# nikkolasg/playsnark

Hardware: AMD Instinct MI355X
Metric: G1 scalar-muls/s (Pippenger MSM, 2^20 pts per GPU) (higher is better)
Workload: dtype i32x14 (381-bit Fp, 28-bit unsaturated limbs, Montgomery); 1 GPU; BLS12-381 G1 MSM, 2^20 points per GPU, uniform 255-bit scalars; points_per_gpu=1048576, window_bits=20, windows=13, window_table=True, window_table_bytes=1744830464, slice=32, in_flight=4

## Files before the change

### include/playsnark_hip.h

```cpp
#ifndef PLAYSNARK_HIP_H
#define PLAYSNARK_HIP_H
#include <stddef.h>
#include <stdint.h>

#ifdef __cplusplus
extern "C" {
#endif

#define PS_OK 0
#define PS_ERR_LENGTH (-1)
#define PS_ERR_NOT_DIVISIBLE (-2)
#define PS_ERR_ENCODING (-3)
#define PS_ERR_HIP (-4)
#define PS_ERR_ARG (-5)
#define PS_ERR_NO_DEVICE (-6)

#define PS_FMT_AFFINE 0
#define PS_FMT_COMPRESSED 1

#define PS_G1 1
#define PS_G2 2

typedef struct ps_ctx ps_ctx;
typedef struct ps_points ps_points;
// ... 50 lines not shown
int ps_points_sum(int group, const uint8_t* pts, size_t k, uint8_t* out);
int ps_points_lincomb(int group, const uint8_t* pts, const uint8_t* scalars_be32, size_t k, uint8_t* out);
int ps_msm_multi_device(ps_ctx* const* ctxs, const ps_points* const* pts, const ps_scalars* const* scalars, size_t ndev, uint8_t* out);
typedef struct {
    int window_bits;
    int windows;
    uint64_t entries;
    uint64_t buckets;
    int slice;
    int window_table;
} ps_msm_info;
int ps_msm_last_info(ps_ctx* ctx, ps_msm_info* out);
int ps_msm_set_window(ps_ctx* ctx, int window_bits );
int ps_msm_set_slice(ps_ctx* ctx, int entries );
int ps_msm_set_tail(ps_ctx* ctx, int mode);
int ps_microbench_mad(ps_ctx* ctx, double* lane_mads_per_s);
#define PS_MSM_STAGES 7
int ps_ctx_set_timing(ps_ctx* ctx, int enable);
int ps_msm_last_stage_ms(ps_ctx* ctx, float ms[PS_MSM_STAGES]);

typedef struct {
    const uint32_t* row_ptr;
    const uint32_t* col;
    const int64_t* val;
} ps_csr;
int ps_qap_create(ps_ctx* ctx, size_t n_gates, size_t n_vars, size_t n_io, const ps_csr* L, const ps_csr* R,
                  const ps_csr* O, ps_qap** out);
void ps_qap_free(ps_qap* q);
typedef struct {
    const uint32_t* row_ptr;
// ... 159 lines not shown
```

### playsnark_amd/_lib.py

```python
from __future__ import annotations

import ctypes as C
import os

from .build import library_path

PS_OK = 0
PS_ERR_LENGTH = -1
PS_ERR_NOT_DIVISIBLE = -2
PS_ERR_ENCODING = -3
PS_ERR_HIP = -4
PS_ERR_ARG = -5
PS_ERR_NO_DEVICE = -6
PS_FMT_AFFINE, PS_FMT_COMPRESSED = 0, 1
PS_G1, PS_G2 = 1, 2

SYMBOLS = [
    "ps_abi_version", "ps_last_error", "ps_version", "ps_device_count",
    "ps_ctx_create", "ps_ctx_destroy", "ps_ctx_sync", "ps_ctx_stream", "ps_ctx_set_tables", "ps_ctx_set_table_budget",
    "ps_points_upload", "ps_points_from_scalars", "ps_points_download", "ps_points_download_fmt", "ps_points_len", "ps_points_group",
    "ps_points_slice", "ps_points_free", "ps_points_check_subgroup", "ps_points_precompute", "ps_points_table_window",
    "ps_scalars_upload", "ps_scalars_upload_i64", "ps_scalars_from_device_be32", "ps_scalars_download",
    "ps_scalars_len", "ps_scalars_slice", "ps_scalars_free",
    "ps_msm", "ps_msm_be32", "ps_msm_i64", "ps_msm_launch", "ps_msm_finish", "ps_msm_multi", "ps_points_sum", "ps_point_convert",
    "ps_msm_last_info", "ps_msm_set_window", "ps_msm_set_slice", "ps_msm_set_tail", "ps_microbench_mad", "ps_ctx_set_timing", "ps_msm_last_stage_ms",
    "ps_qap_create", "ps_qap_free", "ps_qap_quotient", "ps_qap_is_valid", "ps_qap_interpolate", "ps_poly_mul",
    "ps_points_lincomb", "ps_msm_multi_device", "ps_groth16_prove_multi", "ps_points_monomial_to_lagrange",
    "ps_groth16_setup", "ps_phgr13_setup", "ps_phgr13_crs_free", "ps_groth16_prove", "ps_groth16_prove_shard", "ps_groth16_prove_local", "ps_phgr13_prove", "ps_phgr13_prove_shard", "ps_phgr13_prove_multi", "ps_groth16_verify", "ps_phgr13_verify", "ps_pairing_equal", "ps_prove_last_phase_ms",
    "ps_pairing_product_is_one", "ps_groth16_verify_batch", "ps_groth16_verify_batch_locate", "ps_groth16_verify_batch_locate_info",
    "ps_qap_column_sums", "ps_groth16_setup_from_srs", "ps_groth16_crs_contribute", "ps_groth16_crs_check_update",
    "ps_scalars_powers", "ps_groth16_srs_contribute", "ps_groth16_srs_check", "ps_groth16_srs_check_update",
    "ps_points_lagrange_check", "ps_groth16_crs_check_from_srs",
    "ps_qap_create_fr", "ps_qap_wide_entries",
    "ps_msm_batch", "ps_msm_batch_set_chunk", "ps_groth16_prove_batch",
]


PS_MSM_QUEUE = 4


class MsmInfo(C.Structure):
    _fields_ = [("window_bits", C.c_int), ("windows", C.c_int), ("entries", C.c_uint64),
                ("buckets", C.c_uint64), ("slice", C.c_int), ("window_table", C.c_int)]


class VerifyLocateInfo(C.Structure):
    _fields_ = [("checks", C.c_uint32), ("levels", C.c_uint32), ("invalid", C.c_uint32), ("reserved", C.c_uint32)]


# ... 116 lines not shown
    lib.ps_msm.argtypes = [vp, vp, vp, C.c_char_p]
    lib.ps_msm_be32.argtypes = [vp, vp, C.c_char_p, sz, C.c_char_p]
    lib.ps_msm_i64.argtypes = [vp, vp, vp, sz, C.c_char_p]
    lib.ps_msm_launch.argtypes = [vp, vp, vp]
    lib.ps_msm_finish.argtypes = [vp, C.c_char_p]
    lib.ps_msm_multi.argtypes = [vp, C.POINTER(vp), C.c_size_t, vp, C.POINTER(vp)]
    lib.ps_msm_batch.argtypes = [vp, vp, vp, sz, C.c_char_p]
    lib.ps_msm_batch_set_chunk.argtypes = [vp, i]
    lib.ps_points_sum.argtypes = [i, C.c_char_p, sz, C.c_char_p]
    lib.ps_point_convert.argtypes = [i, i, i, C.c_char_p, C.c_char_p]
    lib.ps_msm_last_info.argtypes = [vp, C.POINTER(MsmInfo)]
    lib.ps_msm_set_window.argtypes = [vp, i]
    lib.ps_ctx_set_timing.argtypes = [vp, i]
    lib.ps_msm_set_slice.argtypes = [vp, i]
    lib.ps_msm_set_tail.argtypes = [vp, i]
    lib.ps_microbench_mad.argtypes = [vp, C.POINTER(C.c_double)]
    lib.ps_ctx_set_table_budget.argtypes = [vp, C.c_longlong]
    lib.ps_qap_is_valid.argtypes = [vp, vp, vp, C.POINTER(C.c_int)]
    lib.ps_msm_last_stage_ms.argtypes = [vp, C.POINTER(C.c_float)]
    lib.ps_qap_create.argtypes = [vp, sz, sz, sz, C.POINTER(Csr), C.POINTER(Csr), C.POINTER(Csr), pp]
    lib.ps_qap_create_fr.argtypes = [vp, sz, sz, sz, C.POINTER(CsrFr), C.POINTER(CsrFr), C.POINTER(CsrFr), pp]
    lib.ps_qap_wide_entries.argtypes = [vp, C.POINTER(sz)]
    lib.ps_qap_free.argtypes = [vp]
    lib.ps_qap_free.restype = None
    lib.ps_qap_quotient.argtypes = [vp, vp, vp, pp, pp, pp, pp]
    lib.ps_poly_mul.argtypes = [vp, vp, vp, pp]
    lib.ps_qap_interpolate.argtypes = [vp, vp, vp, i, pp]
    lib.ps_points_lincomb.argtypes = [i, C.c_char_p, C.c_char_p, sz, C.c_char_p]
    lib.ps_points_monomial_to_lagrange.argtypes = [vp, vp, vp, i, C.POINTER(vp)]
    lib.ps_msm_multi_device.argtypes = [C.POINTER(vp), C.POINTER(vp), C.POINTER(vp), sz, C.c_char_p]
# ... 45 lines not shown
```

### playsnark_amd/api.py

```python
from __future__ import annotations

import ctypes as C
import operator
from typing import Iterable, Optional, Sequence

from . import _lib
from ._lib import PS_G1, PS_G2, lib

G1, G2 = PS_G1, PS_G2
R_ORDER = 0x73EDA753299D7D483339D80809A1D80553BDA402FFFE5BFEFFFFFFFF00000001
FMT_AFFINE, FMT_COMPRESSED = _lib.PS_FMT_AFFINE, _lib.PS_FMT_COMPRESSED
_WIRE = {PS_G1: 96, PS_G2: 192}


class PlaysnarkError(RuntimeError):
    def __init__(self, code, msg):
        super().__init__(f"playsnark_hip error {code}: {msg}")
        self.code = code


class LengthMismatch(ValueError):
    """panic(fmt.Sprintf("mismatch of length between poly %d and blinded eval points %d")) algebra.go:351"""


# ... 41 lines not shown
        v = C.c_double(0.0)
        _check(lib.ps_microbench_mad(self._h, C.byref(v)))
        return v.value

    def set_table_budget(self, nbytes: int):
        _check(lib.ps_ctx_set_table_budget(self._h, nbytes))

    def set_slice(self, entries: int):
        _check(lib.ps_msm_set_slice(self._h, entries))

    def set_batch_chunk(self, members: int):
        _check(lib.ps_msm_batch_set_chunk(self._h, members))

    def set_tail(self, mode: int):
        _check(lib.ps_msm_set_tail(self._h, mode))

    STAGES = ("digits", "scan", "scatter", "queue", "accumulate", "fixup", "reduce")

    def set_timing(self, enable: bool):
        _check(lib.ps_ctx_set_timing(self._h, int(enable)))

    def last_stage_ms(self) -> dict:
        ms = (C.c_float * len(self.STAGES))()
        _check(lib.ps_msm_last_stage_ms(self._h, ms))
        return dict(zip(self.STAGES, list(ms)))

    def last_prove_phase_ms(self) -> dict:
        ms = (C.c_float * 4)()
        _check(lib.ps_prove_last_phase_ms(self._h, ms))
        return dict(zip(("quotient", "prep_or_h_sum", "sums", "total"), list(ms)))
# ... 799 lines not shown
```

### playsnark_amd/csrc/capi.hip

```cpp
#include "../../include/playsnark_hip.h"

#include <hip/hip_runtime.h>

#include <algorithm>
#include <atomic>
#include <chrono>
#include <condition_variable>
#include <functional>
#include <mutex>
#include <cstdio>
#include <cstring>
#include <future>
#include <string>
#include <thread>
#include <vector>

#include "msm.hpp"
#include "msm_batch.hpp"
#include "msm_batch_plan.hpp"
#include "quotient.hpp"
#include "lagrange.hpp"
#include "ec_spmv.hpp"
#include "prove_batch.hpp"
#include "share_ranges.hpp"
// ... 44 lines not shown
        if (p) (void)hipFree(p);
        p = nullptr;
        cap = 0;
    }
};

constexpr size_t PS_PINNED_SLOT = 64 * sizeof(Xyzz<Fp2>) + 16;

struct ps_ctx {
    int device = 0;
    hipStream_t stream = nullptr;
    hipStream_t tail = nullptr;
    hipEvent_t ev_acc_local = nullptr, ev_tail_done = nullptr, ev_sort_local = nullptr;
    bool tail_used = false;
    DevBuf counts, offs, bsum, keys, ranks, vals, sorted, buckets, parts, segs, wins, heavy, hparts, coarse;
    DevBuf mb_fold, mb_out;
    int batch_chunk = 0;
    hipEvent_t mb_ev[2] = {nullptr, nullptr};
    DevBuf pb_x, pb_y, pb_small;
    hipEvent_t pb_ev[6] = {nullptr, nullptr, nullptr, nullptr, nullptr, nullptr};
    bool pb_timed = false;
    DevBuf affine_tmp;
    DevBuf staging;
    DevBuf vb_f12, vb_xyzz, vb_rho, vb_cols;
    float vb_ms[6] = {0, 0, 0, 0, 0, 0};
    DevBuf lc_f12, lc_pts, lc_rows, lc_iolp, lc_work;
    ps_verify_locate_info lc_info{0, 0, 0, 0};
    float lc_ms[3] = {0, 0, 0};
    u32 simds = 0;
    struct ps_scalars* up_scalars = nullptr;
// ... 10 lines not shown
    int q_head = 0, q_len = 0;
    bool pending = false;
    ps_ctx *pipe = nullptr, *pipe2 = nullptr, *pipe3 = nullptr, *pipe4 = nullptr, *pipe5 = nullptr;
    hipEvent_t ev_fork = nullptr;
    ps_ctx* last_chain = nullptr;
    ps_ctx* last_timed = nullptr;
    float phase_ms[PS_PROVE_PHASES] = {0, 0, 0, 0};
    bool use_tables = true;
    long long table_budget = -1;
    void* d_small = nullptr;
    hipEvent_t ev_q = nullptr;
    ps_msm_info last_info{};
    int forced_c = 0;
    int forced_slice = 0;
    int forced_tail = 0;
    QuotientCache* qcache = nullptr;
    ps_ctx* aux = nullptr;
    unsigned long long g16_key[4] = {0, 0, 0, 0};
    uint8_t g16_fixed[96 * 3 + 192 * 2] = {0};
    ps_points *g16_pa = nullptr, *g16_pb = nullptr, *g16_pc = nullptr;
    bool g16_tabs = false;
    bool g16_split = false;
    size_t g16_b1_min_n = (size_t)1 << 19;
    bool g16_multi_hsplit = true;
    hipEvent_t g16_ready = nullptr;
    unsigned long long phgr_key[3] = {0, 0, 0};
    ps_points* phgr_bsum = nullptr;
    bool timing = false;
    hipEvent_t ev[PS_MSM_STAGES + 1] = {};
    bool ev_valid = false;
// ... 105 lines not shown
    }
    HIP_TRY(hipMalloc((void**)&c->d_flag, 64));
    c->h_pinned_cap = PS_MSM_MULTI_MAX * PS_PINNED_SLOT + 64;
    HIP_TRY(hipHostMalloc(&c->h_pinned, c->h_pinned_cap));
    for (auto& e : c->ev) HIP_TRY(hipEventCreate(&e));
    *out = c;
    return PS_OK;
}

extern "C" void ps_ctx_destroy(ps_ctx* c) {
    if (!c) return;
    (void)hipSetDevice(c->device);
    (void)hipStreamSynchronize(c->stream);
    if (c->tail) (void)hipStreamSynchronize(c->tail);
    for (DevBuf* b : {&c->counts, &c->offs, &c->bsum, &c->keys, &c->ranks, &c->sorted, &c->buckets, &c->parts,
                      &c->segs, &c->wins, &c->heavy, &c->hparts, &c->vals, &c->coarse, &c->staging, &c->affine_tmp, &c->mb_fold, &c->mb_out, &c->pb_x, &c->pb_y, &c->pb_small, &c->fb_table[0], &c->fb_table[1],
                      &c->vb_f12, &c->vb_xyzz, &c->vb_rho, &c->vb_cols,
                      &c->lc_f12, &c->lc_pts, &c->lc_rows, &c->lc_iolp, &c->lc_work})
        b->release();
    quotient_cache_free(c->qcache);
    if (c->up_scalars) ps_scalars_free(c->up_scalars);
    for (ps_scalars* v : c->pv_scalars)
        if (v) ps_scalars_free(v);
    if (c->g16_pa) ps_points_free(c->g16_pa);
    if (c->g16_pb) ps_points_free(c->g16_pb);
    if (c->g16_pc) ps_points_free(c->g16_pc);
    if (c->g16_ready) (void)hipEventDestroy(c->g16_ready);
    if (c->phgr_bsum) ps_points_free(c->phgr_bsum);
    if (c->aux) ps_ctx_destroy(c->aux);
    if (c->pipe) ps_ctx_destroy(c->pipe);
    if (c->pipe2) ps_ctx_destroy(c->pipe2);
// ... 737 lines not shown
            int bin_shift = 4;
            while ((pl.NB >> bin_shift) > (u32)DIGITS_BINS) bin_shift++;
            hipLaunchKernelGGL(k_digits_grouped, dgrid, dim3(DIGITS_THREADS), 2 * DIGITS_CHUNK * sizeof(u32), st, scalars_ptr(sc),
                               (u32)n, pl.c, pl.W, pl.NB, cadd, bin_shift, fold_neg, single, (u32*)c->counts.p, (u32*)c->keys.p,
                               (u32*)c->vals.p, (u32*)c->ranks.p);
        }
        PS_STAGE_MARK();
        hipLaunchKernelGGL(k_scan_blocks, dim3(scan_tiles), dim3(SCAN_BLOCK), 0, st, (const u32*)c->counts.p, (u32*)c->offs.p,
                           (u32*)c->bsum.p, (u64)G);
        hipLaunchKernelGGL(k_scan_top, dim3(1), dim3(1024), 0, st, (u32*)c->bsum.p, scan_tiles, (u32*)c->offs.p + G);
        hipLaunchKernelGGL(k_scan_add, dim3(scan_tiles), dim3(SCAN_BLOCK), 0, st, (u32*)c->offs.p, (const u32*)c->bsum.p, (u64)G);
        PS_STAGE_MARK();
        hipLaunchKernelGGL(k_scatter, dim3(nblocks(total)), dim3(256), 0, st, (const u32*)c->keys.p, (const u32*)c->vals.p,
                           (const u32*)c->ranks.p, (const u32*)c->offs.p, total, (u32*)c->sorted.p);
    }
    PS_STAGE_MARK();
    HIP_TRY(hipGetLastError());
    if (!pl.qtail) HIP_TRY(hipMemcpyAsync((char*)c->h_pinned + c->h_pinned_cap - 8, (u32*)c->offs.p + G, 4, hipMemcpyDeviceToHost, st));
    return PS_OK;
}

struct TableRef { const char* base; u64 stride; };
static bool table_ref(const ps_points* pts, size_t n, int wbits, int W, TableRef* out) {
    const Storage* st = pts->st;
    const size_t rb = table_row_bytes(pts->group);
    if (const void* t = st->table.load(std::memory_order_acquire)) {
        if (st->table_c == wbits && W <= st->table_W) {
            *out = TableRef{(const char*)t + pts->first * rb, (u64)st->table_stride};
            return true;
        }
// ... 48 lines not shown
    const bool split_fixup = !pl.shortsum;
#endif
    const size_t max_chain = split_fixup ? (size_t)nthreads_acc / 2 + 2 : 0;
    if ((rc = wc->heavy.ensure(4 * (2 * max_heavy + 3 + max_chain)))) return rc;
    const u32 heavy_npb = 256 / QTraits<KF>::GL;
    const size_t max_jobs = (size_t)nthreads_acc / heavy_npb + max_heavy + 1;
    if ((rc = wc->hparts.ensure(sizeof(Xyzz<F>) * max_jobs))) return rc;
    if (!dev_sets && sizeof(Xyzz<F>) * (pl.sets > 1 ? (size_t)pl.sets : (size_t)nres) + 16 > PS_PINNED_SLOT) return fail(PS_ERR_ARG, "too many windows");
    hipStream_t st = wc->stream;
    int evi = 4;
    if (wc->tail_used) HIP_TRY(hipStreamWaitEvent(st, wc->ev_tail_done, 0));
    if (storage_wait_ready(pts->st, st)) return fail(PS_ERR_HIP, "msm: event wait failed");
    if (wait_acc) HIP_TRY(hipStreamWaitEvent(st, wait_acc, 0));
    PS_STAGE_MARK();
    constexpr bool PF = LN == 1 || PS_G2_ACC_WAVES == 1;
    hipLaunchKernelGGL((k_accumulate<KF, PF>), dim3(nblocks((size_t)nthreads_acc * LN)), dim3(256), 0, st, src,
                       (const u32*)c->sorted.p, (const u32*)c->offs.p, (u32)G, pl.M, nthreads_acc, idx_mask, w_stride, pstride,
                       (Xyzz<F>*)wc->buckets.p, (Xyzz<F>*)wc->parts.p, (u32*)wc->heavy.p);
    if (acc_done) HIP_TRY(hipEventRecord(acc_done, st));
    PS_STAGE_MARK();
    HIP_TRY(hipEventRecord(wc->ev_acc_local, st));
    if (!inline_tail) {
        st = wc->tail;
        HIP_TRY(hipStreamWaitEvent(st, wc->ev_acc_local, 0));
    }
    if (pl.shortsum && pl.lpb >= 1) {
        const u32 lpb = qlpb;
        hipLaunchKernelGGL(k_qfixup<KF>, dim3(nblocks(G * (u64)lpb * QTraits<KF>::GL)), dim3(256), 0, st, (const u32*)c->offs.p, (u32)G, pl.M,
                           nthreads_acc, lpb, (const Xyzz<F>*)wc->parts.p, (Xyzz<F>*)wc->buckets.p, (u32*)wc->heavy.p, (u32*)wc->heavy.p + 2);
    } else if (split_fixup) {
        u32* ccount = (u32*)wc->heavy.p + 1;
        u32* clist = (u32*)wc->heavy.p + 2 + 2 * max_heavy + 1;
        hipLaunchKernelGGL(k_fixup_classify<KF>, dim3(nblocks(G * LN)), dim3(256), 0, st, (const u32*)c->offs.p, (u32)G, pl.M, nthreads_acc,
                           (Xyzz<F>*)wc->buckets.p, (u32*)wc->heavy.p, (u32*)wc->heavy.p + 2, ccount, clist);
        if (nthreads_acc > 1)
            hipLaunchKernelGGL(k_fixup_pair<KF>, dim3(nblocks((size_t)(nthreads_acc - 1) * LN)), dim3(256), 0, st, (const u32*)c->offs.p, (u32)G,
                               pl.M, nthreads_acc, (const Xyzz<F>*)wc->parts.p, (Xyzz<F>*)wc->buckets.p);
        constexpr u32 chain_npb = 256 / QTraits<KF>::GL;
        hipLaunchKernelGGL(k_qfixup_chain<KF>, dim3((unsigned)std::min<size_t>((max_chain + chain_npb - 1) / chain_npb, 512)), dim3(256), 0, st,
                           (const u32*)c->offs.p, (u32)G, pl.M, nthreads_acc, (const Xyzz<F>*)wc->parts.p, (Xyzz<F>*)wc->buckets.p,
                           (const u32*)ccount, (const u32*)clist);
    } else
    hipLaunchKernelGGL(k_fixup<KF>, dim3(nblocks(G * LN)), dim3(256), 0, st, (const u32*)c->offs.p, (u32)G, pl.M, nthreads_acc,
                       (const Xyzz<F>*)wc->parts.p, (Xyzz<F>*)wc->buckets.p, (u32*)wc->heavy.p, (u32*)wc->heavy.p + 2);
    {
        const u32* hcount = (const u32*)wc->heavy.p;
        const u32* hlist = hcount + 2;
        u32* job_base = (u32*)wc->heavy.p + 2 + max_heavy;
        hipLaunchKernelGGL(k_heavy_jobs, dim3(1), dim3(256), 0, st, (const u32*)c->offs.p, (u32)G, pl.M, nthreads_acc, hcount, hlist, job_base, heavy_npb);
        hipLaunchKernelGGL(k_qfixup_heavy_part<KF>, dim3(1024), dim3(256), 0, st, (const u32*)c->offs.p, (u32)G, pl.M, nthreads_acc,
                           (const Xyzz<F>*)wc->parts.p,
                           hcount, hlist, (const u32*)job_base, (Xyzz<F>*)wc->hparts.p);
        hipLaunchKernelGGL(k_qfixup_heavy<KF>, dim3(256), dim3(256), 0, st, (const Xyzz<F>*)wc->hparts.p, (Xyzz<F>*)wc->buckets.p, hcount,
                           hlist, (const u32*)job_base);
    }
    PS_STAGE_MARK();
    {
        Xyzz<F>* accs = (Xyzz<F>*)wc->segs.p;
        Xyzz<F>* runs = accs + nseg_total;
        Xyzz<F>* lvl = runs + nseg_total;
// ... 142 lines not shown
        }
    }
    MsmPlan pl = tab ? msm_plan_table(n, max_bits, tab_c) : msm_plan(n, max_bits, c->forced_c);
    if (tab && k == 1) {
        const MsmPlan plain = msm_plan(n, max_bits, 0);
        const double cost_tab = (double)n * pl.W * 10.0 + (double)pl.G * 42.0;
        const double cost_plain = (double)n * plain.W * 10.0 + (double)plain.G * 42.0;
        if (cost_plain < PS_TABLE_COST_MARGIN * cost_tab) pl = plain;
    }
    int plan_group = PS_G1;
    for (size_t i = 0; i < k; i++)
        if (pts[i]->group == PS_G2) plan_group = PS_G2;
    msm_plan_tail(pl, n, plan_group, c->forced_tail, c->q_len > 0);
    if (c->forced_slice) pl.M = c->forced_slice;
    if (pl.shortsum) msm_plan_lpb(pl, n, plan_group);
    if ((u64)pl.W * (u64)n >= (1ull << 32))
        return fail(PS_ERR_ARG, "MSM too long: windows x length = " + std::to_string((u64)pl.W * (u64)n) +
                                    " digits do not fit the 32-bit sort offsets (split the sum, e.g. ps_points_slice)");
    *out = pl;
    return PS_OK;
}

#ifndef PS_MULTI_CHAIN_MIN_ENTRIES
#define PS_MULTI_CHAIN_MIN_ENTRIES (1ull << 40)
#endif
#ifndef PS_CHAIN_MIN_ENTRIES
#define PS_CHAIN_MIN_ENTRIES (1ull << 21)
#endif
static int msm_launch_any(ps_ctx* wc, const ps_points* pts, const ps_scalars* sc, const MsmPlan& pl, hipEvent_t wait_acc,
                          hipEvent_t acc_done, bool inline_tail) {
// ... 39 lines not shown
    } else {
        for (int w = pl.sets - 1; w >= 0; w--) {
            for (int i = 0; i < pl.c; i++) acc = xyzz_dbl<H>(acc);
            xyzz_add<H>(acc, xyzz_to_host<F>(res[w]));
        }
    }
    write_affine(out, acc);
}

static u32 msm_entries(const ps_ctx* c, const MsmPlan& pl, int group) {
    if (!pl.qtail) return *(const u32*)((const char*)c->h_pinned + c->h_pinned_cap - 8);
    const size_t pt = group == PS_G1 ? sizeof(Xyzz<Fp>) : sizeof(Xyzz<Fp2>);
    return *(const u32*)((const char*)c->h_pinned + pt * (pl.sets > 1 ? (size_t)pl.sets : (size_t)pl.c));
}

static void write_identity(int group, uint8_t* out) {
    memset(out, 0, wire_bytes(group));
    out[0] = 0x40;
}

constexpr int PS_MULTI_RING = 4;
static int msm_multi_sort(ps_ctx* c, ps_ctx* const* ring, const ps_scalars* sc, const MsmPlan& pl, bool fork) {
    int rc;
    ps_ctx* w0 = ring[0];
    if (fork) {
        if (!c->ev_fork) HIP_TRY(hipEventCreateWithFlags(&c->ev_fork, hipEventDisableTiming));
        HIP_TRY(hipEventRecord(c->ev_fork, c->stream));
        HIP_TRY(hipStreamWaitEvent(w0->tail, c->ev_fork, 0));
    }
    if ((rc = msm_sort(w0, sc, pl, false, w0->tail))) return rc;
// ... 37 lines not shown
        }
        ring[have++] = *slots[j];
    }
    for (int j = have; j < PS_MULTI_RING; j++) ring[j] = ring[j % have];
    return PS_OK;
}

static int msm_multi_finish(ps_ctx* c, ps_ctx* w0, const ps_points* const* pts, size_t k, const MsmPlan& pl, uint8_t* const* out) {
    for (size_t i = 0; i < k; i++) {
        HIP_TRY(hipEventSynchronize(c->ev_multi[i]));
        if (!out) continue;
        if (pts[i]->group == PS_G1) msm_fold_host<Fp>(w0, pl, (int)i, out[i]);
        else msm_fold_host<Fp2>(w0, pl, (int)i, out[i]);
    }
    c->last_info = ps_msm_info{pl.c, pl.W, msm_entries(w0, pl, pts[0]->group), pl.G, pl.M, pl.table ? 1 : 0};
    return PS_OK;
}

static int msm_multi_check(const char* who, const ps_points* const* pts, size_t k, const ps_scalars* sc) {
    if (k > PS_MSM_MULTI_MAX) return fail(PS_ERR_ARG, std::string(who) + ": more than PS_MSM_MULTI_MAX point arrays");
    for (size_t i = 0; i < k; i++) {
        if (!pts[i]) return fail(PS_ERR_ARG, std::string(who) + ": NULL argument");
        if (pts[i]->n != sc->n)
            return fail(PS_ERR_LENGTH, "mismatch of length between poly " + std::to_string(sc->n) + " and blinded eval points " +
                                           std::to_string(pts[i]->n));
    }
    return PS_OK;
}

extern "C" int ps_msm_multi(ps_ctx* c, const ps_points* const* pts, size_t k, const ps_scalars* sc, uint8_t* const* out) {
// ... 35 lines not shown
        for (int j = 0; j < c->q_len; j++) busy = busy || (cand && c->q[(c->q_head + j) % PS_MSM_QUEUE].wc == cand);
        if (busy) continue;
        if (!cand) {
            int rc = ps_ctx_create(c->device, slots[w]);
            if (rc) return rc;
            cand = *slots[w];
        }
        wc = cand;
    }
    if (!wc) return fail(PS_ERR_ARG, "ps_msm_launch: no free workspace");
    if (wc != c) {
        wc->timing = c->timing;
        wc->forced_c = c->forced_c;
        wc->forced_slice = c->forced_slice;
        wc->forced_tail = c->forced_tail;
    }
    if (!c->ev_fork) HIP_TRY(hipEventCreateWithFlags(&c->ev_fork, hipEventDisableTiming));
    if (c->q_len == 0) HIP_TRY(hipEventRecord(c->ev_fork, c->stream));
    ps_ctx::PendingMsm& e = c->q[(c->q_head + c->q_len) % PS_MSM_QUEUE];
    if (sc->n == 0) {
        e = {pts->group, MsmPlan{}, wc};
    } else {
        MsmPlan pl;
        int rc0 = msm_plan_checked(c, &pts, 1, sc->n, sc->max_bits, &pl);
        if (rc0) return rc0;
        if (wc != c) HIP_TRY(hipStreamWaitEvent(wc->stream, c->ev_fork, 0));
        const bool lone = pl.shortsum && c->q_len == 0;
        if (!lone) HIP_TRY(hipStreamWaitEvent(wc->tail, c->ev_fork, 0));
        const bool chained = (u64)pl.W * sc->n >= PS_CHAIN_MIN_ENTRIES;
        hipEvent_t wait = (chained && c->last_chain && c->last_chain != wc) ? c->last_chain->ev_acc_local : nullptr;
// ... 13 lines not shown
    if (c->q_len == 0) return fail(PS_ERR_ARG, "ps_msm_finish: nothing pending");
    const ps_ctx::PendingMsm e = c->q[c->q_head];
    c->q_head = (c->q_head + 1) % PS_MSM_QUEUE;
    c->q_len--;
    c->pending = c->q_len > 0;
    const MsmPlan& pl = e.plan;
    if (pl.W == 0) {
        write_identity(e.group, out);
        return PS_OK;
    }
    HIP_TRY(hipSetDevice(c->device));
    HIP_TRY(hipEventSynchronize(e.wc->ev_tail_done));
    if (e.group == PS_G1) msm_fold_host<Fp>(e.wc, pl, 0, out);
    else msm_fold_host<Fp2>(e.wc, pl, 0, out);
    c->last_info = ps_msm_info{pl.c, pl.W, msm_entries(e.wc, pl, e.group), pl.G, pl.M, pl.table ? 1 : 0};
    c->last_timed = e.wc;
    return PS_OK;
}

extern "C" int ps_msm(ps_ctx* c, const ps_points* pts, const ps_scalars* sc, uint8_t* out) {
    if (c && c->q_len) return fail(PS_ERR_ARG, "ps_msm: sums are pending on this context (ps_msm_finish them first)");
    int rc = ps_msm_launch(c, pts, sc);
    if (rc) return rc;
    return ps_msm_finish(c, out);
}
extern "C" int ps_msm_be32(ps_ctx* c, const ps_points* pts, const uint8_t* be32, size_t n, uint8_t* out) {
    if (!c || !pts || !out || (n && !be32)) return fail(PS_ERR_ARG, "ps_msm_be32: NULL argument");
    if (c->q_len) return fail(PS_ERR_ARG, "ps_msm: sums are pending on this context (ps_msm_finish them first)");
    if (n >= (1ull << 31)) return fail(PS_ERR_ARG, "vector too long");
    HIP_TRY(hipSetDevice(c->device));
// ... 35 lines not shown
    return scope.finish(ps_msm(c, pts, s, out));
}
extern "C" int ps_msm_last_info(ps_ctx* c, ps_msm_info* out) {
    if (!c || !out) return fail(PS_ERR_ARG, "NULL argument");
    *out = c->last_info;
    return PS_OK;
}
extern "C" int ps_msm_set_slice(ps_ctx* c, int entries) {
    if (!c || entries < 0 || entries > 4096) return fail(PS_ERR_ARG, "slice must be 0 (automatic) or 1..4096");
    c->forced_slice = entries;
    return PS_OK;
}
extern "C" int ps_msm_set_tail(ps_ctx* c, int mode) {
    if (!c || mode < 0 || mode > 2) return fail(PS_ERR_ARG, "tail mode must be 0 (automatic), 1 (chains) or 2 (trees)");
    c->forced_tail = mode;
    return PS_OK;
}
extern "C" int ps_ctx_set_timing(ps_ctx* c, int enable) {
    if (!c) return fail(PS_ERR_ARG, "ctx is NULL");
    c->timing = enable != 0;
    c->ev_valid = false;
    for (ps_ctx* w : {c->pipe, c->pipe2, c->aux, c->pipe3, c->pipe4, c->pipe5})
        if (w) { w->timing = c->timing; w->ev_valid = false; }
    return PS_OK;
}
extern "C" int ps_msm_last_stage_ms(ps_ctx* c, float* ms) {
    if (!c || !ms) return fail(PS_ERR_ARG, "NULL argument");
    const ps_ctx* t = c->last_timed ? c->last_timed : c;
    if (!t->ev_valid) return fail(PS_ERR_ARG, "no timed MSM on this context (ps_ctx_set_timing)");
    HIP_TRY(hipSetDevice(c->device));
// ... 172 lines not shown
```

### playsnark_amd/csrc/msm.hpp

```cpp
#pragma once
#include "curve.hpp"
#include "fixup_class.hpp"

namespace ps {

#ifndef PS_TAIL_PRIO
#define PS_TAIL_PRIO 0
#endif
#if PS_TAIL_PRIO > 0
#define PS_TAIL_PRIO_HERE __builtin_amdgcn_s_setprio(PS_TAIL_PRIO)
#else
#define PS_TAIL_PRIO_HERE do { } while (0)
#endif

struct MsmPlan {
    int c;
    int W;
    u32 NB;
    u64 G;
    int M;
    int SEG;
    int sets;
    bool table;
    bool qtail;
    bool hybrid;
    bool shortsum;
    int lpb;
    int rc_s;
    bool busy;
};
constexpr int ENTRY_W_SHIFT = 26;

static inline MsmPlan msm_plan(size_t n, int max_bits, int forced_c) {
    MsmPlan best{};
    double best_cost = 1e300;
    for (int c = 4; c <= 20; c++) {
        if (forced_c ? c != forced_c : c > 16) continue;
        int W = max_bits / c + 1;
        double nb = (double)(1u << (c - 1));
        double cost = (double)n * W * 10.0 + W * nb * 42.0;
        if (cost < best_cost) {
            best_cost = cost;
            best.c = c;
            best.W = W;
        }
    }
    best.NB = 1u << (best.c - 1);
    best.sets = best.W;
    best.G = (u64)best.W * best.NB;
    best.M = 32;
    const u64 total = (u64)n * best.W;
    while (best.M < 1024 && total / (2 * (u64)best.M) >= (1u << 19)) best.M *= 2;
    while (best.M < 1024 && (u64)best.M * 5 * best.G < total) best.M *= 2;
    while (best.M > 8 && total / (u64)best.M < (1u << 17) && (u64)(best.M / 2) * 5 * best.G >= total) best.M /= 2;
    best.SEG = 8;
    return best;
}
static inline MsmPlan msm_plan_table(size_t n, int max_bits, int c) {
    MsmPlan pl{};
    pl.c = c;
    pl.W = max_bits / c + 1;
    pl.NB = 1u << (c - 1);
    pl.sets = 1;
    pl.table = true;
    pl.G = pl.NB;
    pl.M = 32;
    const u64 total = (u64)n * pl.W;
    while (pl.M < 1024 && total / (2 * (u64)pl.M) >= (1u << 19)) pl.M *= 2;
    while (pl.M < 1024 && (u64)pl.M * 5 * pl.G < total) pl.M *= 2;
    while (pl.M > 8 && total / (u64)pl.M < (1u << 17) && (u64)(pl.M / 2) * 5 * pl.G >= total) pl.M /= 2;
    pl.SEG = 8;
    return pl;
}

PS_INL u32 limb_sel8(const u32* k, int i) {
    u32 v = 0;
#pragma unroll
    for (int j = 0; j < 8; j++) v = (i == j) ? k[j] : v;
    return v;
}
constexpr int DIGITS_THREADS = 1024;
#ifndef PS_DIGITS_PER_THREAD
#define PS_DIGITS_PER_THREAD 8
#endif
constexpr int DIGITS_PER_THREAD = PS_DIGITS_PER_THREAD;
constexpr int DIGITS_CHUNK = DIGITS_THREADS * DIGITS_PER_THREAD;
// ... 632 lines not shown
    }
    g = lo;
    bend = offs[g + 1];
}

#ifndef PS_G2_ACC_WAVES
#define PS_G2_ACC_WAVES 2
#endif
#define PS_ACC_WAVES(KF) (FieldTraits<KF>::LANES == 2 ? PS_G2_ACC_WAVES : 2)
template <class KF, bool PREFETCH>
__global__ void __launch_bounds__(256, PS_ACC_WAVES(KF)) k_accumulate(const char* __restrict__ points,
                                                       const u32* __restrict__ sorted, const u32* __restrict__ offs,
                                                       u32 G, int Mplan, u32 T, u32 idx_mask, u64 w_stride, u32 pstride,
                                                       Xyzz<typename FieldTraits<KF>::Store>* __restrict__ buckets,
                                                       Xyzz<typename FieldTraits<KF>::Store>* __restrict__ parts,
                                                       u32* __restrict__ heavy_count) {
    const u32 E = offs[G];
    const int M = eff_slice(E, T, Mplan);
    const u32 t = logical_tid<KF>();
    if (blockIdx.x == 0 && threadIdx.x == 0) heavy_count[0] = heavy_count[1] = 0;
    const u64 start64 = (u64)t * (u64)M;
    if (start64 >= E) return;
    const u32 start = (u32)start64;
    const u32 end = (E - start < (u32)M) ? E : start + (u32)M;
    u32 lo = 0, hi = G;
    while (hi - lo > 1) {
        u32 mid = (lo + hi) >> 1;
        if (offs[mid] <= start) lo = mid; else hi = mid;
    }
    u32 g = lo;
    u32 bend = offs[g + 1];
// ... 27 lines not shown
                acc = xyzz_identity<KF>();
                run_start = p;
                next_bucket(offs, G, p, g, bend);
            }
            const u32 e = sorted[p];
            Affine<KF> pt = ld_entry_point<KF>(points, e, idx_mask, w_stride, pstride);
            if (!affine_is_identity<KF>(pt)) {
                if (e >> 31) pt.y = f_neg(pt.y);
                xyzz_madd_inl<KF>(acc, pt.x, pt.y);
            }
        }
    }
    flush_run<KF>(acc, g, run_start, end, start, t, offs, buckets, parts);
}


#ifndef PS_TAIL_WAVES
#define PS_TAIL_WAVES 2
#endif

template <class KF>
__global__ void __launch_bounds__(256, PS_TAIL_WAVES) k_fixup(const u32* __restrict__ offs, u32 G, int Mplan, u32 T,
                                                  const Xyzz<typename FieldTraits<KF>::Store>* __restrict__ parts,
                                                  Xyzz<typename FieldTraits<KF>::Store>* __restrict__ buckets,
                                                  u32* __restrict__ heavy_count, u32* __restrict__ heavy_list) {
    PS_TAIL_PRIO_HERE;
    u32 g = logical_tid<KF>();
    if (g >= G) return;
    const int M = eff_slice(offs[G], T, Mplan);
    u32 lo = offs[g], hi = offs[g + 1];
// ... 9 lines not shown
    }
    Xyzz<KF> acc = xyzz_identity<KF>();
    for (u32 t = t0; t <= t1; t++) {
        u32 slice_start = t * (u32)M;
        u32 rs = lo > slice_start ? lo : slice_start;
        Xyzz<KF> part = ld_xyzz<KF>(&parts[2 * (size_t)t + (rs == slice_start ? 0 : 1)]);
        xyzz_add_inl<KF>(acc, part);
    }
    st_xyzz<KF>(&buckets[g], acc);
}

template <class KF>
__global__ void __launch_bounds__(256) k_fixup_classify(const u32* __restrict__ offs, u32 G, int Mplan, u32 T,
                                                        Xyzz<typename FieldTraits<KF>::Store>* __restrict__ buckets,
                                                        u32* __restrict__ heavy_count, u32* __restrict__ heavy_list,
                                                        u32* __restrict__ chain_count, u32* __restrict__ chain_list) {
    PS_TAIL_PRIO_HERE;
    const u32 g = logical_tid<KF>();
    if (g >= G) return;
    const int M = eff_slice(offs[G], T, Mplan);
    const int cls = bucket_class(offs[g], offs[g + 1], (u32)M, HEAVY_SPAN);
    if (cls == BUCKET_EMPTY) {
        st_xyzz<KF>(&buckets[g], xyzz_identity<KF>());
    } else if (cls == BUCKET_CHAIN) {
        if (pair_leader<KF>()) chain_list[atomicAdd(chain_count, 1u)] = g;
    } else if (cls == BUCKET_HEAVY) {
        if (pair_leader<KF>()) heavy_list[atomicAdd(heavy_count, 1u)] = g;
    }
}

template <class KF>
__global__ void __launch_bounds__(256, PS_TAIL_WAVES) k_fixup_pair(const u32* __restrict__ offs, u32 G, int Mplan, u32 T,
                                                       const Xyzz<typename FieldTraits<KF>::Store>* __restrict__ parts,
                                                       Xyzz<typename FieldTraits<KF>::Store>* __restrict__ buckets) {
    PS_TAIL_PRIO_HERE;
    const u32 t = logical_tid<KF>() + 1;
    if (t >= T) return;
    const u32 E = offs[G];
    const int M = eff_slice(E, T, Mplan);
    u32 g;
    if (!pair_boundary_bucket(offs, G, E, t, (u32)M, HEAVY_SPAN, g)) return;
    Xyzz<KF> acc = ld_xyzz<KF>(&parts[part_slot(offs[g], t - 1, (u32)M)]);
    const Xyzz<KF> right = ld_xyzz<KF>(&parts[2 * (size_t)t]);
    xyzz_add_inl<KF>(acc, right);
    st_xyzz<KF>(&buckets[g], acc);
}

constexpr u32 HEAVY_CHUNK = 1024;
__host__ __device__ inline u32 heavy_chunk_of(u32 span, u32 npb) {
    u32 s = 1;
// ... 546 lines not shown
```

Baseline: 433.3 million G1 scalar-muls/s.

## Add whole-bucket accumulation path with size-sorted bucket ordering

```diff
diff --git a/include/playsnark_hip.h b/include/playsnark_hip.h
--- a/include/playsnark_hip.h
+++ b/include/playsnark_hip.h
@@ -88,6 +88,8 @@
 int ps_msm_set_window(ps_ctx* ctx, int window_bits );
 int ps_msm_set_slice(ps_ctx* ctx, int entries );
 int ps_msm_set_tail(ps_ctx* ctx, int mode);
+int ps_msm_set_accumulate(ps_ctx* ctx, int mode);
+int ps_msm_last_accumulate(ps_ctx* ctx, int* path);
 int ps_microbench_mad(ps_ctx* ctx, double* lane_mads_per_s);
 #define PS_MSM_STAGES 7
 int ps_ctx_set_timing(ps_ctx* ctx, int enable);
diff --git a/playsnark_amd/_lib.py b/playsnark_amd/_lib.py
--- a/playsnark_amd/_lib.py
+++ b/playsnark_amd/_lib.py
@@ -33,6 +33,7 @@
     "ps_points_lagrange_check", "ps_groth16_crs_check_from_srs",
     "ps_qap_create_fr", "ps_qap_wide_entries",
     "ps_msm_batch", "ps_msm_batch_set_chunk", "ps_groth16_prove_batch",
+    "ps_msm_set_accumulate", "ps_msm_last_accumulate",
 ]
 
 
@@ -179,6 +180,9 @@
     lib.ps_ctx_set_timing.argtypes = [vp, i]
     lib.ps_msm_set_slice.argtypes = [vp, i]
     lib.ps_msm_set_tail.argtypes = [vp, i]
+    if hasattr(lib, "ps_msm_set_accumulate"):
+        lib.ps_msm_set_accumulate.argtypes = [vp, i]
+        lib.ps_msm_last_accumulate.argtypes = [vp, C.POINTER(C.c_int)]
     lib.ps_microbench_mad.argtypes = [vp, C.POINTER(C.c_double)]
     lib.ps_ctx_set_table_budget.argtypes = [vp, C.c_longlong]
     lib.ps_qap_is_valid.argtypes = [vp, vp, vp, C.POINTER(C.c_int)]
diff --git a/playsnark_amd/api.py b/playsnark_amd/api.py
--- a/playsnark_amd/api.py
+++ b/playsnark_amd/api.py
@@ -79,6 +79,14 @@
 
     def set_tail(self, mode: int):
         _check(lib.ps_msm_set_tail(self._h, mode))
+
+    def set_accumulate(self, mode: int):
+        _check(lib.ps_msm_set_accumulate(self._h, mode))
+
+    def last_accumulate_path(self) -> int:
+        path = C.c_int(0)
+        _check(lib.ps_msm_last_accumulate(self._h, C.byref(path)))
+        return path.value
 
     STAGES = ("digits", "scan", "scatter", "queue", "accumulate", "fixup", "reduce")
 
diff --git a/playsnark_amd/csrc/bucket_order.hpp b/playsnark_amd/csrc/bucket_order.hpp
--- /dev/null
+++ b/playsnark_amd/csrc/bucket_order.hpp
@@ -0,0 +1,41 @@
+#pragma once
+#include "field.hpp"
+
+namespace ps {
+
+constexpr u32 BO_CLASSES = 256;
+constexpr u32 BO_PLACE_ITEMS = 4;
+constexpr u32 BO_PLACE_TILE = 256 * BO_PLACE_ITEMS;
+
+enum AccumulatePath : u32 { ACC_AUTO = 0, ACC_SLICES = 1, ACC_BUCKETS = 2 };
+
+constexpr u64 BO_MIN_BUCKETS = 1ull << 18;
+constexpr u64 BO_MAX_MEAN = 64;
+constexpr int BO_SHORT_BITS = 64;
+inline bool bo_host_admits(bool shortsum, u64 G, u64 digits, int max_bits) {
+    return !shortsum && max_bits > BO_SHORT_BITS && G >= BO_MIN_BUCKETS && digits <= BO_MAX_MEAN * G;
+}
+constexpr u32 BO_EVEN_MULT = 4;
+constexpr u32 BO_EVEN_ADD = 32;
+
+PS_HD inline u32 bo_class(u32 lo, u32 hi) {
+    const u32 s = hi - lo;
+    return s < BO_CLASSES - 1 ? s : BO_CLASSES - 1;
+}
+
+PS_HD inline u32 bo_scan_desc(const u32* hist, u32* start) {
+    u32 run = 0, maxc = 0;
+    for (u32 k = BO_CLASSES; k-- > 0;) {
+        start[k] = run;
+        run += hist[k];
+        if (hist[k] && k > maxc) maxc = k;
+    }
+    return maxc;
+}
+
+PS_HD inline u32 bo_verdict(u32 maxc, u32 nonempty, u32 E) {
+    if (nonempty == 0 || maxc >= BO_CLASSES - 1) return ACC_SLICES;
+    return (u64)maxc * nonempty <= (u64)BO_EVEN_MULT * E + (u64)BO_EVEN_ADD * nonempty ? ACC_BUCKETS : ACC_SLICES;
+}
+
+}
diff --git a/playsnark_amd/csrc/capi.hip b/playsnark_amd/csrc/capi.hip
--- a/playsnark_amd/csrc/capi.hip
+++ b/playsnark_amd/csrc/capi.hip
@@ -82,6 +82,7 @@
     hipEvent_t ev_acc_local = nullptr, ev_tail_done = nullptr, ev_sort_local = nullptr;
     bool tail_used = false;
     DevBuf counts, offs, bsum, keys, ranks, vals, sorted, buckets, parts, segs, wins, heavy, hparts, coarse;
+    DevBuf perm, border;
     DevBuf mb_fold, mb_out;
     int batch_chunk = 0;
     hipEvent_t mb_ev[2] = {nullptr, nullptr};
@@ -122,6 +123,8 @@
     int forced_c = 0;
     int forced_slice = 0;
     int forced_tail = 0;
+    int forced_acc = 0;
+    int last_acc = 0;
     QuotientCache* qcache = nullptr;
     ps_ctx* aux = nullptr;
     unsigned long long g16_key[4] = {0, 0, 0, 0};
@@ -257,7 +260,7 @@
     (void)hipStreamSynchronize(c->stream);
     if (c->tail) (void)hipStreamSynchronize(c->tail);
     for (DevBuf* b : {&c->counts, &c->offs, &c->bsum, &c->keys, &c->ranks, &c->sorted, &c->buckets, &c->parts,
-                      &c->segs, &c->wins, &c->heavy, &c->hparts, &c->vals, &c->coarse, &c->staging, &c->affine_tmp, &c->mb_fold, &c->mb_out, &c->pb_x, &c->pb_y, &c->pb_small, &c->fb_table[0], &c->fb_table[1],
+                      &c->segs, &c->wins, &c->heavy, &c->hparts, &c->vals, &c->coarse, &c->perm, &c->border, &c->staging, &c->affine_tmp, &c->mb_fold, &c->mb_out, &c->pb_x, &c->pb_y, &c->pb_small, &c->fb_table[0], &c->fb_table[1],
                       &c->vb_f12, &c->vb_xyzz, &c->vb_rho, &c->vb_cols,
                       &c->lc_f12, &c->lc_pts, &c->lc_rows, &c->lc_iolp, &c->lc_work})
         b->release();
@@ -1025,6 +1028,20 @@
         hipLaunchKernelGGL(k_scatter, dim3(nblocks(total)), dim3(256), 0, st, (const u32*)c->keys.p, (const u32*)c->vals.p,
                            (const u32*)c->ranks.p, (const u32*)c->offs.p, total, (u32*)c->sorted.p);
     }
+    if (pl.acc != ACC_SLICES) {
+        if ((rc = c->perm.ensure(4 * G))) return rc;
+        if ((rc = c->border.ensure(4 * (2 * (size_t)BO_CLASSES + 4)))) return rc;
+        u32* hist = (u32*)c->border.p;
+        u32* cursors = hist + BO_CLASSES;
+        u32* verdict = cursors + BO_CLASSES;
+        const unsigned tiles = (unsigned)((G + BO_PLACE_TILE - 1) / BO_PLACE_TILE);
+        HIP_TRY(hipMemsetAsync(hist, 0, 4 * BO_CLASSES, st));
+        hipLaunchKernelGGL(k_bo_count, dim3(tiles), dim3(256), 0, st, (const u32*)c->offs.p, (u32)G, hist);
+        hipLaunchKernelGGL(k_bo_scan, dim3(1), dim3(BO_CLASSES), 0, st, (const u32*)hist, (const u32*)c->offs.p, (u32)G, (u32)pl.acc, cursors,
+                           verdict);
+        hipLaunchKernelGGL(k_bo_place, dim3(tiles), dim3(256), 0, st, (const u32*)c->offs.p, (u32)G, cursors, (u32*)c->perm.p);
+        HIP_TRY(hipMemcpyAsync((char*)c->h_pinned + c->h_pinned_cap - 16, verdict, 4, hipMemcpyDeviceToHost, st));
+    }
     PS_STAGE_MARK();
     HIP_TRY(hipGetLastError());
     if (!pl.qtail) HIP_TRY(hipMemcpyAsync((char*)c->h_pinned + c->h_pinned_cap - 8, (u32*)c->offs.p + G, 4, hipMemcpyDeviceToHost, st));
@@ -1103,9 +1120,16 @@
     if (wait_acc) HIP_TRY(hipStreamWaitEvent(st, wait_acc, 0));
     PS_STAGE_MARK();
     constexpr bool PF = LN == 1 || PS_G2_ACC_WAVES == 1;
+    const u32 acc_mode = dev_sets ? (u32)ACC_SLICES : (u32)pl.acc;
+    const u32* verdict = acc_mode == ACC_SLICES ? nullptr : (const u32*)c->border.p + 2 * BO_CLASSES;
+    if (acc_mode != ACC_SLICES)
+        hipLaunchKernelGGL((k_bucket_sum<KF, PF>), dim3(nblocks(G * LN)), dim3(256), 0, st, src, (const u32*)c->sorted.p,
+                           (const u32*)c->offs.p, (const u32*)c->perm.p, (u32)G, idx_mask, w_stride, pstride, (Xyzz<F>*)wc->buckets.p,
+                           (u32*)wc->heavy.p, verdict);
+    if (acc_mode != ACC_BUCKETS)
     hipLaunchKernelGGL((k_accumulate<KF, PF>), dim3(nblocks((size_t)nthreads_acc * LN)), dim3(256), 0, st, src,
                        (const u32*)c->sorted.p, (const u32*)c->offs.p, (u32)G, pl.M, nthreads_acc, idx_mask, w_stride, pstride,
-                       (Xyzz<F>*)wc->buckets.p, (Xyzz<F>*)wc->parts.p, (u32*)wc->heavy.p);
+                       (Xyzz<F>*)wc->buckets.p, (Xyzz<F>*)wc->parts.p, (u32*)wc->heavy.p, verdict);
     if (acc_done) HIP_TRY(hipEventRecord(acc_done, st));
     PS_STAGE_MARK();
     HIP_TRY(hipEventRecord(wc->ev_acc_local, st));
@@ -1113,7 +1137,8 @@
         st = wc->tail;
         HIP_TRY(hipStreamWaitEvent(st, wc->ev_acc_local, 0));
     }
-    if (pl.shortsum && pl.lpb >= 1) {
+    if (acc_mode == ACC_BUCKETS) {
+    } else if (pl.shortsum && pl.lpb >= 1) {
         const u32 lpb = qlpb;
         hipLaunchKernelGGL(k_qfixup<KF>, dim3(nblocks(G * (u64)lpb * QTraits<KF>::GL)), dim3(256), 0, st, (const u32*)c->offs.p, (u32)G, pl.M,
                            nthreads_acc, lpb, (const Xyzz<F>*)wc->parts.p, (Xyzz<F>*)wc->buckets.p, (u32*)wc->heavy.p, (u32*)wc->heavy.p + 2);
@@ -1121,10 +1146,10 @@
         u32* ccount = (u32*)wc->heavy.p + 1;
         u32* clist = (u32*)wc->heavy.p + 2 + 2 * max_heavy + 1;
         hipLaunchKernelGGL(k_fixup_classify<KF>, dim3(nblocks(G * LN)), dim3(256), 0, st, (const u32*)c->offs.p, (u32)G, pl.M, nthreads_acc,
-                           (Xyzz<F>*)wc->buckets.p, (u32*)wc->heavy.p, (u32*)wc->heavy.p + 2, ccount, clist);
+                           (Xyzz<F>*)wc->buckets.p, (u32*)wc->heavy.p, (u32*)wc->heavy.p + 2, ccount, clist, verdict);
         if (nthreads_acc > 1)
             hipLaunchKernelGGL(k_fixup_pair<KF>, dim3(nblocks((size_t)(nthreads_acc - 1) * LN)), dim3(256), 0, st, (const u32*)c->offs.p, (u32)G,
-                               pl.M, nthreads_acc, (const Xyzz<F>*)wc->parts.p, (Xyzz<F>*)wc->buckets.p);
+                               pl.M, nthreads_acc, (const Xyzz<F>*)wc->parts.p, (Xyzz<F>*)wc->buckets.p, verdict);
         constexpr u32 chain_npb = 256 / QTraits<KF>::GL;
         hipLaunchKernelGGL(k_qfixup_chain<KF>, dim3((unsigned)std::min<size_t>((max_chain + chain_npb - 1) / chain_npb, 512)), dim3(256), 0, st,
                            (const u32*)c->offs.p, (u32)G, pl.M, nthreads_acc, (const Xyzz<F>*)wc->parts.p, (Xyzz<F>*)wc->buckets.p,
@@ -1132,7 +1157,7 @@
     } else
     hipLaunchKernelGGL(k_fixup<KF>, dim3(nblocks(G * LN)), dim3(256), 0, st, (const u32*)c->offs.p, (u32)G, pl.M, nthreads_acc,
                        (const Xyzz<F>*)wc->parts.p, (Xyzz<F>*)wc->buckets.p, (u32*)wc->heavy.p, (u32*)wc->heavy.p + 2);
-    {
+    if (acc_mode != ACC_BUCKETS) {
         const u32* hcount = (const u32*)wc->heavy.p;
         const u32* hlist = hcount + 2;
         u32* job_base = (u32*)wc->heavy.p + 2 + max_heavy;
@@ -1305,6 +1330,7 @@
     msm_plan_tail(pl, n, plan_group, c->forced_tail, c->q_len > 0);
     if (c->forced_slice) pl.M = c->forced_slice;
     if (pl.shortsum) msm_plan_lpb(pl, n, plan_group);
+    pl.acc = c->forced_acc ? c->forced_acc : bo_host_admits(pl.shortsum, pl.G, (u64)pl.W * n, max_bits) ? (int)ACC_AUTO : (int)ACC_SLICES;
     if ((u64)pl.W * (u64)n >= (1ull << 32))
         return fail(PS_ERR_ARG, "MSM too long: windows x length = " + std::to_string((u64)pl.W * (u64)n) +
                                     " digits do not fit the 32-bit sort offsets (split the sum, e.g. ps_points_slice)");
@@ -1374,6 +1400,10 @@
     return *(const u32*)((const char*)c->h_pinned + pt * (pl.sets > 1 ? (size_t)pl.sets : (size_t)pl.c));
 }
 
+static int msm_acc_path(const ps_ctx* c, const MsmPlan& pl) {
+    return pl.acc != ACC_AUTO ? pl.acc : (int)*(const u32*)((const char*)c->h_pinned + c->h_pinned_cap - 16);
+}
+
 static void write_identity(int group, uint8_t* out) {
     memset(out, 0, wire_bytes(group));
     out[0] = 0x40;
@@ -1441,6 +1471,7 @@
         else msm_fold_host<Fp2>(w0, pl, (int)i, out[i]);
     }
     c->last_info = ps_msm_info{pl.c, pl.W, msm_entries(w0, pl, pts[0]->group), pl.G, pl.M, pl.table ? 1 : 0};
+    c->last_acc = msm_acc_path(w0, pl);
     return PS_OK;
 }
 
@@ -1506,6 +1537,7 @@
         wc->forced_c = c->forced_c;
         wc->forced_slice = c->forced_slice;
         wc->forced_tail = c->forced_tail;
+        wc->forced_acc = c->forced_acc;
     }
     if (!c->ev_fork) HIP_TRY(hipEventCreateWithFlags(&c->ev_fork, hipEventDisableTiming));
     if (c->q_len == 0) HIP_TRY(hipEventRecord(c->ev_fork, c->stream));
@@ -1549,6 +1581,7 @@
     if (e.group == PS_G1) msm_fold_host<Fp>(e.wc, pl, 0, out);
     else msm_fold_host<Fp2>(e.wc, pl, 0, out);
     c->last_info = ps_msm_info{pl.c, pl.W, msm_entries(e.wc, pl, e.group), pl.G, pl.M, pl.table ? 1 : 0};
+    c->last_acc = msm_acc_path(e.wc, pl);
     c->last_timed = e.wc;
     return PS_OK;
 }
@@ -1614,6 +1647,16 @@
 extern "C" int ps_msm_set_tail(ps_ctx* c, int mode) {
     if (!c || mode < 0 || mode > 2) return fail(PS_ERR_ARG, "tail mode must be 0 (automatic), 1 (chains) or 2 (trees)");
     c->forced_tail = mode;
+    return PS_OK;
+}
+extern "C" int ps_msm_set_accumulate(ps_ctx* c, int mode) {
+    if (!c || mode < 0 || mode > 2) return fail(PS_ERR_ARG, "accumulate mode must be 0 (automatic), 1 (slices) or 2 (whole buckets)");
+    c->forced_acc = mode;
+    return PS_OK;
+}
+extern "C" int ps_msm_last_accumulate(ps_ctx* c, int* path) {
+    if (!c || !path) return fail(PS_ERR_ARG, "NULL argument");
+    *path = c->last_acc;
     return PS_OK;
 }
 extern "C" int ps_ctx_set_timing(ps_ctx* c, int enable) {
diff --git a/playsnark_amd/csrc/msm.hpp b/playsnark_amd/csrc/msm.hpp
--- a/playsnark_amd/csrc/msm.hpp
+++ b/playsnark_amd/csrc/msm.hpp
@@ -1,6 +1,7 @@
 #pragma once
 #include "curve.hpp"
 #include "fixup_class.hpp"
+#include "bucket_order.hpp"
 
 namespace ps {
 
@@ -28,6 +29,7 @@
     int lpb;
     int rc_s;
     bool busy;
+    int acc;
 };
 constexpr int ENTRY_W_SHIFT = 26;
 
@@ -54,6 +56,7 @@
     while (best.M < 1024 && (u64)best.M * 5 * best.G < total) best.M *= 2;
     while (best.M > 8 && total / (u64)best.M < (1u << 17) && (u64)(best.M / 2) * 5 * best.G >= total) best.M /= 2;
     best.SEG = 8;
+    best.acc = ACC_SLICES;
     return best;
 }
 static inline MsmPlan msm_plan_table(size_t n, int max_bits, int c) {
@@ -70,6 +73,7 @@
     while (pl.M < 1024 && (u64)pl.M * 5 * pl.G < total) pl.M *= 2;
     while (pl.M > 8 && total / (u64)pl.M < (1u << 17) && (u64)(pl.M / 2) * 5 * pl.G >= total) pl.M /= 2;
     pl.SEG = 8;
+    pl.acc = ACC_SLICES;
     return pl;
 }
 
@@ -732,7 +736,8 @@
                                                        u32 G, int Mplan, u32 T, u32 idx_mask, u64 w_stride, u32 pstride,
                                                        Xyzz<typename FieldTraits<KF>::Store>* __restrict__ buckets,
                                                        Xyzz<typename FieldTraits<KF>::Store>* __restrict__ parts,
-                                                       u32* __restrict__ heavy_count) {
+                                                       u32* __restrict__ heavy_count, const u32* __restrict__ verdict) {
+    if (verdict && *verdict == ACC_BUCKETS) return;
     const u32 E = offs[G];
     const int M = eff_slice(E, T, Mplan);
     const u32 t = logical_tid<KF>();
@@ -790,6 +795,114 @@
     flush_run<KF>(acc, g, run_start, end, start, t, offs, buckets, parts);
 }
 
+__global__ void __launch_bounds__(256) k_bo_count(const u32* __restrict__ offs, u32 G, u32* __restrict__ hist) {
+    PS_TAIL_PRIO_HERE;
+    __shared__ u32 lh[BO_CLASSES];
+    const u32 tid = threadIdx.x;
+    lh[tid] = 0;
+    __syncthreads();
+    const u32 base = blockIdx.x * BO_PLACE_TILE;
+#pragma unroll
+    for (u32 j = 0; j < BO_PLACE_ITEMS; j++) {
+        const u32 g = base + j * 256 + tid;
+        const bool act = g < G;
+        lds_count(lh, act ? bo_class(offs[g], offs[g + 1]) : 0u, act);
+    }
+    __syncthreads();
+    if (lh[tid]) atomicAdd(&hist[tid], lh[tid]);
+}
+__global__ void __launch_bounds__(BO_CLASSES) k_bo_scan(const u32* __restrict__ hist, const u32* __restrict__ offs, u32 G, u32 forced,
+                                                        u32* __restrict__ cursors, u32* __restrict__ out) {
+    PS_TAIL_PRIO_HERE;
+    __shared__ u32 lh[BO_CLASSES], ls[BO_CLASSES];
+    __shared__ u32 maxc_s;
+    const u32 tid = threadIdx.x;
+    lh[tid] = hist[tid];
+    __syncthreads();
+    if (tid == 0) maxc_s = bo_scan_desc(lh, ls);
+    __syncthreads();
+    cursors[tid] = ls[tid];
+    if (tid == 0) {
+        const u32 nonempty = G - lh[0];
+        out[0] = forced != ACC_AUTO ? forced : bo_verdict(maxc_s, nonempty, offs[G]);
+        out[1] = maxc_s;
+        out[2] = nonempty;
+    }
+}
+__global__ void __launch_bounds__(256) k_bo_place(const u32* __restrict__ offs, u32 G, u32* __restrict__ cursors, u32* __restrict__ perm) {
+    PS_TAIL_PRIO_HERE;
+    __shared__ u32 lh[BO_CLASSES];
+    const u32 tid = threadIdx.x;
+    lh[tid] = 0;
+    __syncthreads();
+    const u32 base = blockIdx.x * BO_PLACE_TILE;
+    u32 cls[BO_PLACE_ITEMS];
+#pragma unroll
+    for (u32 j = 0; j < BO_PLACE_ITEMS; j++) {
+        const u32 g = base + j * 256 + tid;
+        const bool act = g < G;
+        cls[j] = act ? bo_class(offs[g], offs[g + 1]) : 0u;
+        lds_count(lh, cls[j], act);
+    }
+    __syncthreads();
+    const u32 cnt = lh[tid];
+    __syncthreads();
+    lh[tid] = cnt ? atomicAdd(&cursors[tid], cnt) : 0u;
+    __syncthreads();
+#pragma unroll
+    for (u32 j = 0; j < BO_PLACE_ITEMS; j++) {
+        const u32 g = base + j * 256 + tid;
+        const bool act = g < G;
+        const u32 pos = lds_rank(lh, cls[j], act);
+        if (act) perm[pos] = g;
+    }
+}
+
+template <class KF, bool PREFETCH>
+__global__ void __launch_bounds__(256, PS_ACC_WAVES(KF)) k_bucket_sum(const char* __restrict__ points, const u32* __restrict__ sorted,
+                                                       const u32* __restrict__ offs, const u32* __restrict__ perm, u32 G,
+                                                       u32 idx_mask, u64 w_stride, u32 pstride,
+                                                       Xyzz<typename FieldTraits<KF>::Store>* __restrict__ buckets,
+                                                       u32* __restrict__ heavy_count, const u32* __restrict__ verdict) {
+    if (*verdict != ACC_BUCKETS) return;
+    if (blockIdx.x == 0 && threadIdx.x == 0) heavy_count[0] = heavy_count[1] = 0;
+    const u32 t = logical_tid<KF>();
+    if (t >= G) return;
+    const u32 g = perm[t];
+    const u32 start = offs[g], end = offs[g + 1];
+    Xyzz<KF> acc = xyzz_identity<KF>();
+    if (start < end) {
+        if (PREFETCH) {
+            u32 e = sorted[start];
+            u32 e1 = start + 1 < end ? sorted[start + 1] : e;
+            Affine<KF> pt = ld_entry_point<KF>(points, e, idx_mask, w_stride, pstride);
+            for (u32 p = start; p < end; p++) {
+                Affine<KF> nxt = pt;
+                u32 e2 = e1;
+                if (p + 1 < end) nxt = ld_entry_point<KF>(points, e1, idx_mask, w_stride, pstride);
+                if (p + 2 < end) e2 = sorted[p + 2];
+                if (!affine_is_identity<KF>(pt)) {
+                    if (e >> 31) pt.y = f_neg(pt.y);
+                    if (p == start) acc = xyzz_from_affine<KF>(pt.x, pt.y);
+                    else xyzz_madd_inl<KF>(acc, pt.x, pt.y);
+                }
+                pt = nxt; e = e1; e1 = e2;
+            }
+        } else {
+            for (u32 p = start; p < end; p++) {
+                const u32 e = sorted[p];
+                Affine<KF> pt = ld_entry_point<KF>(points, e, idx_mask, w_stride, pstride);
+                if (!affine_is_identity<KF>(pt)) {
+                    if (e >> 31) pt.y = f_neg(pt.y);
+                    if (p == start) acc = xyzz_from_affine<KF>(pt.x, pt.y);
+                    else xyzz_madd_inl<KF>(acc, pt.x, pt.y);
+                }
+            }
+        }
+    }
+    st_xyzz<KF>(&buckets[g], acc);
+}
+
 
 #ifndef PS_TAIL_WAVES
 #define PS_TAIL_WAVES 2
@@ -829,8 +942,10 @@
 __global__ void __launch_bounds__(256) k_fixup_classify(const u32* __restrict__ offs, u32 G, int Mplan, u32 T,
                                                         Xyzz<typename FieldTraits<KF>::Store>* __restrict__ buckets,
                                                         u32* __restrict__ heavy_count, u32* __restrict__ heavy_list,
-                                                        u32* __restrict__ chain_count, u32* __restrict__ chain_list) {
+                                                        u32* __restrict__ chain_count, u32* __restrict__ chain_list,
+                                                        const u32* __restrict__ verdict) {
     PS_TAIL_PRIO_HERE;
+    if (verdict && *verdict == ACC_BUCKETS) return;
     const u32 g = logical_tid<KF>();
     if (g >= G) return;
     const int M = eff_slice(offs[G], T, Mplan);
@@ -847,8 +962,10 @@
 template <class KF>
 __global__ void __launch_bounds__(256, PS_TAIL_WAVES) k_fixup_pair(const u32* __restrict__ offs, u32 G, int Mplan, u32 T,
                                                        const Xyzz<typename FieldTraits<KF>::Store>* __restrict__ parts,
-                                                       Xyzz<typename FieldTraits<KF>::Store>* __restrict__ buckets) {
+                                                       Xyzz<typename FieldTraits<KF>::Store>* __restrict__ buckets,
+                                                       const u32* __restrict__ verdict) {
     PS_TAIL_PRIO_HERE;
+    if (verdict && *verdict == ACC_BUCKETS) return;
     const u32 t = logical_tid<KF>() + 1;
     if (t >= T) return;
     const u32 E = offs[G];
```

Result: faster. 450.5 million G1 scalar-muls/s, median of 6 (+4.0%).
